# google/zopfli

Measured on AMD Instinct MI355X. Metric: input MB/s at numiterations=15 (gzip, bit-exact vs reference), higher is better.
Workload: dtype u8 (f32/f64 cost DP); 1 GPU; class-T synthetic (text-like, the enwik8 stand-in) 100000000 B per GPU, numiterations=15, blocksplitting=0, gzip, BASELINE configs[1]; total_bytes=100000000, master_blocks=100, gather=none (one rank)

## Files before the change

### zopfli_amd/csrc/device/drv_build.h

```cpp
#pragma once

constexpr u32 kMatchGrid = 1024;
constexpr u32 kMatchGrid5 = 1536;

extern "C" {
static unsigned SegL(u64 total_positions) {
  if (Knobs().seg_l_set) return Knobs().seg_l;
  total_positions = std::max<u64>(total_positions, zamd::CallPositions());
  return total_positions <= (128u << 10) ? 256u : total_positions <= (16u << 20) ? 512u : total_positions <= (48u << 20) ? 1024u : 2048u;
}
static unsigned SegHead(size_t nb) {
  const unsigned v = Knobs().seg_head;
  return v ? v : (nb >= 48 ? 8192u : 0u);
}


static int LayoutBlocks(zmx_ctx* c, const zmx_block* blocks, size_t nb, zmx_tables* t, u64* la_total, u64* max_window) {
  t->nb = nb;
  t->blocks.resize(nb);
  t->bsize.resize(nb);
  t->store_begin[0].assign(nb, 0);
  t->store_begin[1].assign(nb, 0);
  std::vector<u32> tile_off(nb + 1, 0);
  u64 pos_off = 0, reg_off = 0, la_off = 0, max_l = 0;
  for (size_t b = 0; b < nb; ++b) {
    if (blocks[b].inend < blocks[b].instart || blocks[b].inend > c->insize) {
      return FailMsg("zmx_tables_build: block outside the resident input");
    }
    BlockDesc& d = t->blocks[b];
    d.instart = blocks[b].instart;
    d.inend = blocks[b].inend;
    d.ws = d.instart > ZMX_WINDOW ? d.instart - ZMX_WINDOW : 0;
    if (!c->seg_starts.empty()) {
      const size_t k = static_cast<size_t>(std::upper_bound(c->seg_starts.begin(), c->seg_starts.end(), d.instart) -
                                           c->seg_starts.begin()) - 1;
      const u64 seg_end = k + 1 < c->seg_starts.size() ? c->seg_starts[k + 1] : c->insize;
      if (d.inend > seg_end) return FailMsg("zmx_tables_build: block spans two input segments (zmx_set_input_segments)");
      d.ws = std::max<u64>(d.ws, c->seg_starts[k]);
    }
    d.pos_off = pos_off;
    d.reg_off = reg_off;
    d.la_off = la_off;
    const u64 B = d.inend - d.instart, L = d.inend - d.ws;
    if (B > 0x7fff0000ull) return FailMsg("zmx_tables_build: block too large (positions are 32-bit)");
    t->bsize[b] = static_cast<u32>(B);
    pos_off += B;
    reg_off += (L + 7) & ~7ull;
    la_off += (B + 1 + 7) & ~7ull;
    max_l = std::max(max_l, L);
    tile_off[b + 1] = tile_off[b] + static_cast<u32>((B + MT - 1) / MT);
  }
  t->total_b = pos_off;
  t->total_l = reg_off;
  t->tile_off = tile_off;
  *la_total = la_off;
  *max_window = max_l;
  return 0;
}

struct ReusePlan {
  bool reuse = false;
  std::vector<u64> src_pos;
  std::vector<u64> link_lo;
  std::vector<u32> tile_list;
};
static ReusePlan PlanReuse(const zmx_ctx* c, const zmx_tables* t, const zmx_tables* parent, const std::vector<uint64_t>& tail_r) {
  const size_t nb = t->nb;
  const u64 pos_off = t->total_b;
  const std::vector<u32>& tile_off = t->tile_off;
  ReusePlan plan;
  bool reuse = parent != nullptr && parent->nb > 0 && (c->h_in != nullptr || tail_r.size() == nb) && parent->d_recs != nullptr &&
               parent->total_b + pos_off < (3ull << 30);
  if (reuse) {
    plan.src_pos.resize(nb);
    plan.link_lo.resize(nb);
    size_t pb = 0;
    for (size_t b = 0; b < nb && reuse; ++b) {
      const BlockDesc& d = t->blocks[b];
      while (pb < parent->nb && parent->blocks[pb].inend < d.inend) ++pb;
      if (pb == parent->nb || d.instart < parent->blocks[pb].instart || d.inend > parent->blocks[pb].inend) {
        reuse = false;
        break;
      }
      const BlockDesc& pd = parent->blocks[pb];
      plan.src_pos[b] = pd.pos_off + (d.instart - pd.instart);
      const u64 B = d.inend - d.instart;
      plan.link_lo[b] = d.inend - d.ws;
      if (B == 0 || d.inend == pd.inend) continue;
      u64 t0 = B > ZMX_MAX_MATCH ? d.inend - ZMX_MAX_MATCH : d.instart;
      const u64 r = c->h_in ? zamd::TailRunStart(c->h_in, d.instart, d.inend) : tail_r[b];
      if (r < t0) t0 = r;
      const u32 tile_first = static_cast<u32>((t0 - d.instart) / MT);
      for (u32 tile = tile_first; tile < tile_off[b + 1] - tile_off[b]; ++tile) {
        plan.tile_list.push_back(tile_off[b] + tile);
      }
      const u64 first_index = d.instart + static_cast<u64>(tile_first) * MT - d.ws;
      plan.link_lo[b] = first_index > ZMX_WINDOW ? first_index - ZMX_WINDOW : 0;
    }
  }
  plan.reuse = reuse;
  return plan;
}

static int TailRuns(zmx_ctx* c, const zmx_tables* t, std::vector<uint64_t>* r) {
  const size_t nb = t->nb;
  std::vector<uint64_t> blocks(2 * nb);
  for (size_t b = 0; b < nb; ++b) {
    blocks[2 * b] = t->blocks[b].instart;
    blocks[2 * b + 1] = t->blocks[b].inend;
  }
  PoolScope tmp(c);
  uint64_t* d_blocks = nullptr;
  uint64_t* d_r = nullptr;
  HIPCHK(tmp.Upload(&d_blocks, blocks.data(), 2 * nb, "d_blocks"));
  HIPCHK(tmp.AllocT(&d_r, nb, "d_r"));
  TailRunParams P;
  P.in = c->d_in;
  P.blocks = d_blocks;
  P.r = d_r;
  hipLaunchKernelGGL(k_tail_runs, dim3(static_cast<unsigned>(nb)), dim3(64), 0, c->stream, P);
  KCHK(c, "k_tail_runs");
  r->resize(nb);
  HIPCHK(hipMemcpyAsync(r->data(), d_r, nb * sizeof(uint64_t), hipMemcpyDeviceToHost, c->stream));
  HIPCHK(hipStreamSynchronize(c->stream));
  return 0;
}

static int AllocTableArrays(zmx_ctx* c, zmx_tables* t, u64 la_off) {
  const size_t nb = t->nb;
  const u64 pos_off = t->total_b;
  const u64 reg_off = t->total_l;
  const std::vector<u32>& tile_off = t->tile_off;
  HIPCHK(PoolAlloc(c, &t->d_blocks, nb));
  HIPCHK(PoolAlloc(c, &t->d_tile_off, nb + 1));
  HIPCHK(PoolAlloc(c, &t->d_same16, reg_off));
  HIPCHK(PoolAlloc(c, &t->d_links, reg_off));
  HIPCHK(PoolAlloc(c, &t->d_recs, pos_off * 8));
  HIPCHK(PoolAlloc(c, &t->d_la, la_off));
  HIPCHK(PoolAlloc(c, &t->d_store[0], pos_off));
  HIPCHK(PoolAlloc(c, &t->d_store[1], pos_off));
  t->run = RunLayout(nb);
  HIPCHK(PoolAlloc(c, &t->d_runin, t->run.in_bytes));
  HIPCHK(PoolAlloc(c, &t->d_runout, t->run.out_bytes));
  HIPCHK(c->pool.PinnedTake(&t->h_runin, t->run.in_bytes, &t->h_runin_cap));
  HIPCHK(c->pool.PinnedTake(&t->h_runout, t->run.out_bytes, &t->h_runout_cap));
  HIPCHK(hipMemsetAsync(t->run.stats(t->d_runout), 0, RunLayout::stats_and_flags_bytes(), c->stream));
  HIPCHK(PoolAlloc(c, &t->d_dph, pos_off));
  HIPCHK(PoolAlloc(c, &t->d_block_edges, nb));
  t->badpos_words = pos_off / 32 + 4;
  HIPCHK(PoolAlloc(c, &t->d_badpos, t->badpos_words));
  HIPCHK(PoolAlloc(c, &t->d_code_base, nb));
  HIPCHK(PoolAlloc(c, &t->d_wtab, nb * ZMX_WTAB));
  HIPCHK(PoolAlloc(c, &t->d_badcodes, nb * 40));
  HIPCHK(PoolAlloc(c, &t->d_counters, 48));
  HIPCHK(hipMemcpyAsync(t->d_blocks, t->blocks.data(), nb * sizeof(BlockDesc), hipMemcpyHostToDevice, c->stream));
  HIPCHK(hipMemcpyAsync(t->d_tile_off, tile_off.data(), (nb + 1) * sizeof(u32), hipMemcpyHostToDevice, c->stream));
  HIPCHK(hipMemsetAsync(t->run.flags(t->d_runout), 0, RunLayout::kFlags * sizeof(u32), c->stream));
  return 0;
}

struct MatchBuild {
  PoolScope hash_tmp;
  u16* d_lev = nullptr;
  u16* d_tot2 = nullptr;
  u16* d_rank2 = nullptr;
  uint4* d_xrec = nullptr;
  u32* d_tot12 = nullptr;
  unsigned long long* d_energy = nullptr;
  u32* d_cmax = nullptr;
  u8* d_est = nullptr;
  bool skip_any = false, skip_all = false;
  double skip_positions = 0;
  unsigned long long* d_m5stats = nullptr;
  bool join_stream2 = false;
  explicit MatchBuild(zmx_ctx* c) : hash_tmp(c) {}
};

static int LaunchHash(zmx_ctx* c, zmx_tables* t, int mk, u64 max_l, const u64* d_link_lo, MatchBuild& m) {
  const size_t nb = t->nb;
  const u64 reg_off = t->total_l;
  if (max_l == 0) return 0;
  const dim3 g1(static_cast<unsigned>((max_l + 256 * SAME_CH - 1) / (256 * SAME_CH)), static_cast<unsigned>(nb));
  hipLaunchKernelGGL(k_same, g1, dim3(256), 0, c->stream, c->d_in, t->d_blocks, t->d_same16, d_link_lo);
  KCHK(c, "k_same");
  const dim3 g2(static_cast<unsigned>((max_l + CH_EMIT - 1) / CH_EMIT), static_cast<unsigned>(nb), 2);
  hipLaunchKernelGGL(k_chain, g2, dim3(64), CH_LDS_BYTES, c->stream, c->d_in, t->d_blocks, t->d_same16, t->d_links, d_link_lo);
  KCHK(c, "k_chain");
  const bool walks = mk == 5 || mk == 0;
  const bool order = mk != 5 && MatchOrder();
  if ((walks || order) && d_link_lo == nullptr) {
    m.skip_any = mk == 5;
    if (mk == 5) for (size_t b = 0; b < nb; ++b) m.skip_positions += static_cast<double>(t->blocks[b].inend - t->blocks[b].instart);
    const unsigned hits_chunks = static_cast<unsigned>((max_l + RK_CH - 1) / RK_CH);
    {
      if (!m.d_energy) HIPCHK(m.hash_tmp.AllocT(&m.d_energy, nb, "d_energy"));
      if (walks && !m.d_cmax) HIPCHK(m.hash_tmp.AllocT(&m.d_cmax, nb * static_cast<size_t>(hits_chunks) + 1, "d_cmax"));
      if (order && !m.d_est) HIPCHK(m.hash_tmp.AllocT(&m.d_est, reg_off, "d_est"));
      HIPCHK(hipMemsetAsync(m.d_energy, 0, nb * sizeof(unsigned long long), c->stream));
      if (m.d_cmax) HIPCHK(hipMemsetAsync(m.d_cmax, 0, (nb * static_cast<size_t>(hits_chunks) + 1) * sizeof(u32), c->stream));
      HitsParams hp;
      hp.in = c->d_in;
      hp.blocks = t->d_blocks;
      hp.same16 = t->d_same16;
      hp.energy = m.d_energy;
      hp.cmax = m.d_cmax;
      hp.est = m.d_est;
      const dim3 g5(hits_chunks, static_cast<unsigned>(nb));
      hipLaunchKernelGGL(k_hits, g5, dim3(RK_THREADS), 0, c->stream, hp);
      KCHK(c, "k_hits");
    }
    if (!walks) return 0;
    if (mk == 0) {
      std::vector<unsigned long long> energy(nb);
      HIPCHK(hipMemcpyAsync(energy.data(), m.d_energy, nb * sizeof(unsigned long long), hipMemcpyDeviceToHost, c->stream));
      HIPCHK(hipStreamSynchronize(c->stream));
      size_t on = 0;
      for (size_t b = 0; b < nb; ++b) {
        if (energy[b] > Knobs().match_hits * (t->blocks[b].inend - t->blocks[b].ws)) {
          ++on;
          m.skip_positions += static_cast<double>(t->blocks[b].inend - t->blocks[b].instart);
        }
      }
      m.skip_any = on != 0;
      m.skip_all = on == nb;
    }
    if (m.skip_any) {
      if (!m.d_lev) HIPCHK(m.hash_tmp.AllocT(&m.d_lev, static_cast<size_t>(LV_N) * reg_off, "d_lev"));
      if (!m.d_tot2) HIPCHK(m.hash_tmp.AllocT(&m.d_tot2, 2 * reg_off, "d_tot"));
      if (!m.d_rank2) HIPCHK(m.hash_tmp.AllocT(&m.d_rank2, 2 * reg_off, "d_rank"));
      if (!m.d_tot12) HIPCHK(m.hash_tmp.AllocT(&m.d_tot12, reg_off, "d_tot12"));
      if (!m.d_xrec) HIPCHK(m.hash_tmp.AllocT(&m.d_xrec, 2 * reg_off, "d_xrec"));
      LevelParams lp;
      lp.in = c->d_in;
      lp.blocks = t->d_blocks;
      lp.lev = m.d_lev;
      lp.total_l = reg_off;
      lp.energy = mk == 0 ? m.d_energy : nullptr;
      lp.thr = Knobs().match_hits;
      const dim3 g4(static_cast<unsigned>((max_l + LV_CH - 1) / LV_CH), static_cast<unsigned>(nb), LV_N);
      hipLaunchKernelGGL(k_levels, g4, dim3(64), 0, c->stream, lp);
      KCHK(c, "k_levels");
      RankParams rp;
      rp.in = c->d_in;
      rp.blocks = t->d_blocks;
      rp.links = t->d_links;
      rp.same16 = t->d_same16;
      rp.lev = m.d_lev;
      rp.total_l = reg_off;
      rp.tot = m.d_tot2;
      rp.rank = m.d_rank2;
      rp.xrec = m.d_xrec;
      rp.tot12 = m.d_tot12;
      rp.energy = lp.energy;
      rp.thr = lp.thr;
      rp.cmax = m.d_cmax;
      rp.cmax_stride = hits_chunks;
      const dim3 g3(static_cast<unsigned>((max_l + RK_CH - 1) / RK_CH), static_cast<unsigned>(nb));
      hipLaunchKernelGGL(k_rank2, g3, dim3(RK_THREADS), 0, c->stream, rp);
      KCHK(c, "k_rank2");
    }
  }
  return 0;
}
static int BuildHashLinks(zmx_ctx* c, zmx_tables* t, int mk, u64 max_l, const ReusePlan& plan, MatchBuild& m) {
  const size_t nb = t->nb;
  HIPCHK(hipEventRecord(c->ev[0], c->stream));
  u64* d_link_lo = nullptr;
  if (plan.reuse) HIPCHK(m.hash_tmp.Upload(&d_link_lo, plan.link_lo.data(), nb, "d_link_lo"));
  if (LaunchHash(c, t, mk, max_l, d_link_lo, m) != 0) return -1;
  t->links_partial = plan.reuse;
  return 0;
}

static int LaunchMatch(zmx_ctx* c, zmx_tables* t, int mk, MatchBuild& m, u32* pool, u32 pool_cap, u32 total_tiles, const u32* d_tiles, bool prof) {
  const size_t nb = t->nb;
  if (total_tiles == 0) return 0;
  MatchParams mp;
  mp.in = c->d_in;
  mp.blocks = t->d_blocks;
  mp.tile_off = t->d_tile_off;
  mp.nb = static_cast<u32>(nb);
  mp.total_tiles = total_tiles;
  mp.links = t->d_links;
  mp.recs = t->d_recs;
  mp.pool = pool;
  mp.pool_cap = pool_cap;
  mp.counters = t->d_counters;
  mp.scratch = c->d_scratch;
  mp.tile_list = d_tiles;
  mp.skip_energy = nullptr;
  mp.skip_thr = 0;
  mp.est = d_tiles == nullptr ? m.d_est : nullptr;
  if ((mk == 5 || mk == 0) && d_tiles == nullptr && m.skip_any) {
    if (!c->d_scratch5) HIPCHK(PoolAllocT(c, &c->d_scratch5, static_cast<size_t>(kMatchGrid5) * M5_THREADS * SCRATCH_CPS, "d_scratch5"));
    Match5Params q;
    q.m = mp;
    q.m.scratch = c->d_scratch5;
    q.xrec = m.d_xrec;
    q.tot12 = m.d_tot12;
    q.energy = mk == 0 ? m.d_energy : nullptr;
    q.thr = Knobs().match_hits;
    const size_t m5_waves = static_cast<size_t>(kMatchGrid5) * (M5_THREADS / 64);
    if (!m.d_m5stats) HIPCHK(m.hash_tmp.AllocT(&m.d_m5stats, 2 * m5_waves, "d_m5stats"));
    HIPCHK(hipMemsetAsync(m.d_m5stats, 0, 2 * m5_waves * sizeof(unsigned long long), c->stream));
    q.wave_stats = m.d_m5stats;
    {
      const u64 waves = static_cast<u64>(kMatchGrid5) * (M5_THREADS / 64);
      q.sub_shift = mp.total_tiles >= 4 * waves ? 1u : 2u;
    }
    if (mk == 5 || m.skip_all) {
      hipLaunchKernelGGL(k_match5, dim3(kMatchGrid5), dim3(M5_THREADS), 0, c->stream, q);
      KCHK(c, "k_match5");
      return 0;
    }
    HIPCHK(hipEventRecord(c->ev2[0], c->stream));
    HIPCHK(hipStreamWaitEvent(c->stream2, c->ev2[0], 0));
    hipLaunchKernelGGL(k_match5, dim3(kMatchGrid5), dim3(M5_THREADS), 0, c->stream2, q);
    HIPCHK(hipGetLastError());
    c->stream2_outstanding = true;
    HIPCHK(hipEventRecord(c->ev2[1], c->stream2));
    m.join_stream2 = true;
    mp.skip_energy = m.d_energy;
    mp.skip_thr = Knobs().match_hits;
  }
  const bool filt = Knobs().match_filter;
  if (prof && filt) hipLaunchKernelGGL((k_match2<true, true>), dim3(kMatchGrid), dim3(M2_THREADS), 0, c->stream, mp);
  else if (prof) hipLaunchKernelGGL((k_match2<true, false>), dim3(kMatchGrid), dim3(M2_THREADS), 0, c->stream, mp);
  else if (filt) hipLaunchKernelGGL((k_match2<false, true>), dim3(kMatchGrid), dim3(M2_THREADS), 0, c->stream, mp);
  else hipLaunchKernelGGL((k_match2<false, false>), dim3(kMatchGrid), dim3(M2_THREADS), 0, c->stream, mp);
  if (m.join_stream2) {
    m.join_stream2 = false;
    HIPCHK(hipStreamWaitEvent(c->stream, c->ev2[1], 0));
    c->stream2_outstanding = false;
  }
  KCHK(c, "k_match2");
  return 0;
}

static int BuildMatchRecords(zmx_ctx* c, zmx_tables* t, zmx_tables* parent, int mk, u64 max_l, const ReusePlan& plan, MatchBuild& m) {
  const size_t nb = t->nb;
  const u64 pos_off = t->total_b;
  const std::vector<u32>& tile_off = t->tile_off;
  bool reuse = plan.reuse;
  if (!c->d_scratch) HIPCHK(PoolAllocT(c, &c->d_scratch, static_cast<size_t>(kMatchGrid) * M2_THREADS * SCRATCH_CPS, "d_scratch"));
  HIPCHK(hipEventRecord(c->ev[1], c->stream));
  double match_positions = 0;
  double m5_lane_iters = 0, m5_iters = 0;
  if (reuse) {
    u64* d_src_pos = nullptr;
    u32* d_tile_list = nullptr;
    PoolScope tmp(c);
    HIPCHK(tmp.Upload(&d_src_pos, plan.src_pos.data(), nb, "d_src_pos"));
    HIPCHK(tmp.Upload(&d_tile_list, plan.tile_list.data(), plan.tile_list.size(), "d_tile_list"));
    CopyRecsParams cp;
    cp.blocks = t->d_blocks;
    cp.src_pos = d_src_pos;
    cp.src = reinterpret_cast<const uint4*>(parent->d_recs);
    cp.dst = reinterpret_cast<uint4*>(t->d_recs);
    u64 max_b = 0;
    for (size_t b = 0; b < nb; ++b) max_b = std::max<u64>(max_b, t->bsize[b]);
    const unsigned gx = static_cast<unsigned>(std::min<u64>(std::max<u64>((max_b * 2 + 256 * 16 - 1) / (256 * 16), 1), 4096));
    hipLaunchKernelGGL(k_copy_recs, dim3(gx, static_cast<unsigned>(nb)), dim3(256), 0, c->stream, cp);
    KCHK(c, "k_copy_recs");
    HIPCHK(hipMemsetAsync(t->d_counters, 0, 48 * sizeof(u32), c->stream));
    HIPCHK(hipMemcpyAsync(t->d_counters, parent->d_counters, sizeof(u32), hipMemcpyDeviceToDevice, c->stream));
    if (LaunchMatch(c, t, mk, m, parent->d_pool, parent->pool_cap, static_cast<u32>(plan.tile_list.size()), d_tile_list, false) != 0) return -1;
    u32 counters[2] = {0, 0};
    HIPCHK(hipMemcpyAsync(counters, t->d_counters, sizeof(counters), hipMemcpyDeviceToHost, c->stream));
    HIPCHK(hipStreamSynchronize(c->stream));
    if ((counters[1] & 1u) == 0) {
      t->d_pool = parent->d_pool;
      t->pool_cap = parent->pool_cap;
      parent->d_pool = nullptr;
      parent->pool_cap = 0;
      parent->params.trace.pool = nullptr;
    } else {
      reuse = false;
      if (LaunchHash(c, t, mk, max_l, nullptr, m) != 0) return -1;
      t->links_partial = false;
    }
  }

  const u64 pool_entries = Knobs().pool_entries;
  u64 per_pos = 4;
  for (bool first_try = true; !reuse; first_try = false) {
    u64 cap = std::max<u64>(pos_off * per_pos, 1u << 16);
    if (first_try && pool_entries) cap = pool_entries;
    if (cap > 0xfffffff0ull) cap = 0xfffffff0ull;
    PoolFree(c, t->d_pool);
    t->d_pool = nullptr;
    HIPCHK(PoolAlloc(c, &t->d_pool, cap));
    t->pool_cap = static_cast<u32>(cap);
    HIPCHK(hipMemsetAsync(t->d_counters, 0, 48 * sizeof(u32), c->stream));
    if (LaunchMatch(c, t, mk, m, t->d_pool, t->pool_cap, tile_off[nb], nullptr, Knobs().prof) != 0) return -1;
    u32 counters[2] = {0, 0};
    HIPCHK(hipMemcpyAsync(counters, t->d_counters, sizeof(counters), hipMemcpyDeviceToHost, c->stream));
    HIPCHK(hipStreamSynchronize(c->stream));
    match_positions += static_cast<double>(pos_off);
    if (m.d_m5stats) {
      const size_t m5_waves = static_cast<size_t>(kMatchGrid5) * (M5_THREADS / 64);
      std::vector<unsigned long long> ws(2 * m5_waves);
      HIPCHK(hipMemcpy(ws.data(), m.d_m5stats, ws.size() * sizeof(unsigned long long), hipMemcpyDeviceToHost));
      m5_lane_iters = m5_iters = 0;
      for (size_t w = 0; w < m5_waves; ++w) { m5_lane_iters += static_cast<double>(ws[2 * w]); m5_iters += static_cast<double>(ws[2 * w + 1]); }
    }
    if (counters[1] & 2u) {
      u32 dbg[8] = {0};
      HIPCHK(hipMemcpy(dbg, t->d_counters + 32, sizeof(dbg), hipMemcpyDeviceToHost));
      char buf[320];
      std::snprintf(buf, sizeof(buf), "zmx_tables_build: k_match5's wave loop did not end (state %08x xd %u curd %u bestlen %u limit %u nlink %u eqd %u "
                    "li %u idx %u same %u cur %u bestdist %u)", dbg[0], dbg[1], dbg[2], dbg[3] & 0xffffu, dbg[3] >> 16, dbg[4] & 0xffffu, dbg[4] >> 16,
                    dbg[5], dbg[6] & 0xffffu, dbg[6] >> 16, dbg[7] & 0xffffu, dbg[7] >> 16);
      return FailFault(buf);
    }
    if ((counters[1] & 1u) == 0) break;
    if (per_pos >= 256) return FailMsg("zmx_tables_build: change-point pool overflow");
    per_pos *= 8;
  }
  {
    HIPCHK(hipEventRecord(c->ev[2], c->stream));
    HIPCHK(hipEventSynchronize(c->ev[2]));
    float ms_hash = 0, ms_match = 0;
    HIPCHK(hipEventElapsedTime(&ms_hash, c->ev[0], c->ev[1]));
    HIPCHK(hipEventElapsedTime(&ms_match, c->ev[1], c->ev[2]));
    zmx_stats& ts = zamd::ThreadStats();
    ts.match[0] += ms_match * 1e-3;
    ts.match[1] += ms_hash * 1e-3;
    ts.match[2] += 1;
    ts.match[3] += reuse ? static_cast<double>(plan.tile_list.size()) * MT : match_positions;
    if (m.skip_any && !reuse) {
      ts.match5[0] += m5_lane_iters;
      ts.match5[1] += m5_iters;
      ts.match5[2] += m.skip_positions;
    }
    if (Knobs().prof && !reuse) {
      unsigned long long hc[2] = {0, 0};
      HIPCHK(hipMemcpy(hc, t->d_counters + 4, sizeof(hc), hipMemcpyDeviceToHost));
      const double pos = static_cast<double>(pos_off);
      std::fprintf(stderr, "%s: %.2f ms for %.0f positions: %.1f chain hits per "
                   "position, %.1f of 64 lanes with a hit per wave-loop iteration; %.1f SIMD cycles per hit (2.4 GHz, 1024 SIMDs)\n", mk == 5 || mk == 0 ? "k_match5 / k_match2 (hits = entries touched)" : "k_match2", ms_match, pos,
                   static_cast<double>(hc[0]) / pos, static_cast<double>(hc[0]) / static_cast<double>(hc[1] ? hc[1] : 1),
                   ms_match * 1e-3 * 2.4e9 * 1024 / static_cast<double>(hc[0] ? hc[0] : 1));
      if (mk != 5) {
        int wgs = 0;
        if (Knobs().match_filter) HIPCHK(hipOccupancyMaxActiveBlocksPerMultiprocessor(&wgs, k_match2<false, true>, M2_THREADS, 0));
        else HIPCHK(hipOccupancyMaxActiveBlocksPerMultiprocessor(&wgs, k_match2<false, false>, M2_THREADS, 0));
        std::fprintf(stderr, "k_match2: %d workgroups of %u threads resident per CU; positions handed out %s\n", wgs, M2_THREADS,
                     m.d_est ? "by k_hits' estimate, longest first" : "in ascending order");
      }
    }
  }
  return 0;
}

static int BuildDpRows(zmx_ctx* c, zmx_tables* t) {
  const size_t nb = t->nb;
  const std::vector<u32>& tile_off = t->tile_off;
  RowScanParams rp;
  rp.blocks = t->d_blocks;
  rp.recs = t->d_recs;
  rp.dph = t->d_dph;
  rp.block_edges = t->d_block_edges;
  rp.codeless = !Knobs().run_codes && SegL(t->total_b) != 0 ? 1u : 0u;
  hipLaunchKernelGGL(k_rowscan, dim3(static_cast<unsigned>(nb)), dim3(1024), 0, c->stream, rp);
  KCHK(c, "k_rowscan");
  t->block_edges.resize(nb);
  HIPCHK(hipMemcpyAsync(t->block_edges.data(), t->d_block_edges, nb * sizeof(u64), hipMemcpyDeviceToHost, c->stream));
  HIPCHK(hipStreamSynchronize(c->stream));
  {
    const u64 env_mb = Knobs().code_budget_mb;
    const u64 budget = (env_mb ? env_mb * (1ull << 20) : static_cast<u64>(c->code_budget)) / sizeof(u16);
    std::vector<u64> code_base(nb, 0);
    u64 cur = 0;
    for (size_t b = 0; b < nb; ++b) {
      if (t->block_edges[b] > 0xffff0000ull) return FailMsg("zmx_tables_build: block too large (DP row offsets are 32-bit)");
      code_base[b] = cur;
      cur += ((t->block_edges[b] + DP_PIECE - 1) & ~static_cast<u64>(DP_PIECE - 1)) + DP_PIECE;
    }
    if (cur > budget && nb > 1) {
      return FailTooLarge("zmx_tables_build: the batch needs more room for its DP edges than ZOPFLI_AMD_CODE_BUDGET_MB allows");
    }
    HIPCHK(PoolAlloc(c, &t->d_codes, cur + 2048));
    HIPCHK(hipMemcpyAsync(t->d_code_base, code_base.data(), nb * sizeof(u64), hipMemcpyHostToDevice, c->stream));
    CodeParams kp;
    kp.blocks = t->d_blocks;
    kp.tile_off = t->d_tile_off;
    kp.nb_total = static_cast<u32>(nb);
    kp.recs = t->d_recs;
    kp.pool = t->d_pool;
// ... 312 lines not shown
```

### zopfli_amd/csrc/device/zmx_kernels.h

```cpp
#pragma once
#include <hip/hip_runtime.h>
#include <stdint.h>

#include "zmx_record.h"

typedef unsigned char u8;
typedef unsigned short u16;
typedef unsigned int u32;
typedef unsigned long long u64;

struct BlockDesc {
  u64 instart, inend, ws;
  u64 pos_off;
  u64 reg_off;
  u64 la_off;
};

#define ZMX_WINDOW 32768u
#define ZMX_MAX_MATCH 258u
#define ZMX_MAX_CHAIN_HITS 8192
#define ZMX_NONE16 0xffffu

__device__ __forceinline__ int dev_dist_symbol(u32 d) {
  if (d < 5) return (int)d - 1;
  const int l = 31 - __clz((int)(d - 1));
  return 2 * l + (int)(((d - 1) >> (l - 1)) & 1);
}
__device__ __forceinline__ int dev_dist_extra_bits(u32 d) {
  return d < 5 ? 0 : (31 - __clz((int)(d - 1))) - 1;
}
__device__ __forceinline__ int dev_length_symbol(u32 l) {
  if (l < 11) return 254 + (int)l;
  if (l == 258) return 285;
  const int e = 31 - __clz((int)(l - 3)) - 2;
  return 261 + 4 * e + (int)(((l - 3) >> e) & 3);
}
__device__ __forceinline__ int dev_length_extra_bits(u32 l) {
  if (l < 11 || l == 258) return 0;
  return 31 - __clz((int)(l - 3)) - 2;
}

__device__ __forceinline__ u32 find_block(const u32* off, u32 n, u32 x) {
  u32 lo = 0, hi = n;
  while (hi - lo > 1) {
    const u32 mid = (lo + hi) >> 1;
    if (off[mid] <= x) lo = mid; else hi = mid;
  }
  return lo;
}

#define ZMX_WAVE_SCAN(NAME, OP, IDENT)                                                   \
  __device__ __forceinline__ u32 NAME(u32 v) {                                           \
    u32 t;                                                                               \
    t = (u32)__builtin_amdgcn_update_dpp((int)(IDENT), (int)v, 0x111, 0xf, 0xf, false); v = OP(v, t); \
    t = (u32)__builtin_amdgcn_update_dpp((int)(IDENT), (int)v, 0x112, 0xf, 0xf, false); v = OP(v, t); \
    t = (u32)__builtin_amdgcn_update_dpp((int)(IDENT), (int)v, 0x114, 0xf, 0xf, false); v = OP(v, t); \
    t = (u32)__builtin_amdgcn_update_dpp((int)(IDENT), (int)v, 0x118, 0xf, 0xf, false); v = OP(v, t); \
    t = (u32)__builtin_amdgcn_update_dpp((int)(IDENT), (int)v, 0x142, 0xa, 0xf, false); v = OP(v, t); \
    t = (u32)__builtin_amdgcn_update_dpp((int)(IDENT), (int)v, 0x143, 0xc, 0xf, false); v = OP(v, t); \
    return v;                                                                            \
  }
__device__ __forceinline__ u32 zmx_addu(u32 a, u32 b) { return a + b; }
__device__ __forceinline__ u32 zmx_maxu(u32 a, u32 b) { return a > b ? a : b; }
ZMX_WAVE_SCAN(wave_scan_add, zmx_addu, 0u)
ZMX_WAVE_SCAN(wave_scan_max, zmx_maxu, 0u)

__device__ __forceinline__ u32 rdlane_u32(u32 v, u32 l) { return (u32)__builtin_amdgcn_readlane((int)v, (int)l); }
__device__ __forceinline__ float rdlane_f32(float v, u32 l) {
  return __int_as_float(__builtin_amdgcn_readlane(__float_as_int(v), (int)l));
}
__device__ __forceinline__ void wave_lds_sync() {
  __builtin_amdgcn_fence(__ATOMIC_ACQ_REL, "wavefront");
  __builtin_amdgcn_wave_barrier();
}

#define SAME_CH 64

__global__ __launch_bounds__(256) void k_same(const u8* __restrict__ in, const BlockDesc* __restrict__ blocks,
                                              u16* __restrict__ same16, const u64* __restrict__ link_lo) {
  const BlockDesc bd = blocks[blockIdx.y];
  const u64 L = bd.inend - bd.ws;
  const u64 c0 = ((u64)blockIdx.x * blockDim.x + threadIdx.x) * SAME_CH;
  if (c0 >= L) return;
  const u64 c1 = (c0 + SAME_CH < L) ? c0 + SAME_CH : L;
  if (link_lo) {
    const u64 lo = link_lo[blockIdx.y];
    if (lo >= L) return;
    const u64 chunk0 = lo / 32768u * 32768u;
    if (c1 + 32768u <= chunk0) return;
  }
  const u8* base = in + bd.ws;
  u32 next = 0;
  if (c1 < L) {
    const u8 c = base[c1];
    u64 q = c1 + 1;
    u32 r = 0;
    bool stop = false;
    while (q < L && r < 65535u && (((u64)(base + q)) & 7)) {
      if (base[q] != c) { stop = true; break; }
      ++q; ++r;
    }
    if (!stop) {
      const u64 pat = 0x0101010101010101ull * c;
      while (q + 8 <= L && r < 65535u) {
        const u64 x = *reinterpret_cast<const u64*>(base + q) ^ pat;
        if (x) { r += (u32)(__ffsll((long long)x) - 1) >> 3; stop = true; break; }
        q += 8; r += 8;
      }
      if (!stop) {
        while (q < L && r < 65535u && base[q] == c) { ++q; ++r; }
      }
    }
    next = r < 65535u ? r : 65535u;
  }
  u16* out = same16 + bd.reg_off;
  for (u64 k = c1; k-- > c0;) {
    u32 s = 0;
    if (k + 1 < L && base[k + 1] == base[k]) s = next < 65535u ? next + 1 : 65535u;
    out[k] = (u16)s;
    next = s;
  }
}

#define CH_EMIT 32768u
#define CH_TILE 1024u
#define CH_LDS_BYTES (65536 + CH_TILE * 4)

__global__ __launch_bounds__(64) void k_chain(const u8* __restrict__ in, const BlockDesc* __restrict__ blocks,
                                              const u16* __restrict__ same16, ushort4* __restrict__ links,
                                              const u64* __restrict__ link_lo) {
  extern __shared__ __align__(16) u8 dyn_lds[];
  u16* head = reinterpret_cast<u16*>(dyn_lds);
  u16* keys = head + 32768;
  u16* sames = keys + CH_TILE;

  const BlockDesc bd = blocks[blockIdx.y];
  const u32 chain = blockIdx.z;
  const u64 L = bd.inend - bd.ws;
  const u64 e0 = (u64)blockIdx.x * CH_EMIT;
  if (e0 >= L) return;
  const u64 e1 = (e0 + CH_EMIT < L) ? e0 + CH_EMIT : L;
  if (link_lo && e1 <= link_lo[blockIdx.y]) return;
  const u64 w0 = e0 >= ZMX_WINDOW ? e0 - ZMX_WINDOW : 0;
  const u32 lane = threadIdx.x;
  const u64 lt_mask = (1ull << lane) - 1;
  const u64 gt_mask = ~((2ull << lane) - 1);

  for (u32 i = lane; i < 16384; i += 64) reinterpret_cast<u32*>(head)[i] = 0xffffffffu;
  __syncthreads();

  const u8* base = in + bd.ws;
  const u16* same = same16 + bd.reg_off;
  ushort4* lk = links + bd.reg_off;

  for (u64 t0 = w0; t0 < e1; t0 += CH_TILE) {
    const u32 tn = (u32)((e1 - t0 < CH_TILE) ? e1 - t0 : CH_TILE);
    {
      const u32 i0 = 16u * lane;
      u32 by[18];
      u32 sm[16];
#pragma unroll
      for (u32 q = 0; q < 18; ++q) {
        const u64 k = t0 + i0 + q;
        by[q] = (i0 < tn && k < L) ? (u32)base[k] : 0u;
      }
#pragma unroll
      for (u32 q = 0; q < 16; ++q) sm[q] = (i0 + q < tn) ? (u32)same[t0 + i0 + q] : 0u;
#pragma unroll
      for (u32 q = 0; q < 16; ++q) {
        if (i0 + q < tn) {
          u32 v = ((by[q] << 10) ^ (by[q + 1] << 5) ^ by[q + 2]) & 32767u;
          if (chain) v ^= (sm[q] - 3u) & 255u;
          keys[i0 + q] = (u16)v;
          sames[i0 + q] = (u16)sm[q];
        }
      }
    }
    __syncthreads();
    const u32 cur0 = (u32)(t0 - w0);
    for (u32 i0 = 0; i0 < tn; i0 += 64) {
      const u32 i = i0 + lane;
      const bool act = i < tn;
      const u32 key = act ? (u32)keys[i] : 0u;
      if (t0 + i0 + 64 <= e0) {
        const u32 r = cur0 + i;
        bool todo = act;
        while (__any(todo)) {
          if (todo) head[key] = (u16)r;
          wave_lds_sync();
          const u32 w = act ? (u32)head[key] : 0xffffu;
          wave_lds_sync();
          todo = act && w < r;
        }
        continue;
      }
      const u32 old = act ? (u32)head[key] : (u32)ZMX_NONE16;
      u64 grp = __ballot(act);
#pragma unroll
      for (int bit = 0; bit < 15; ++bit) {
        const bool mine = (key >> bit) & 1;
        const u64 bm = __ballot(mine);
        grp &= mine ? bm : ~bm;
      }
      const u64 lower = grp & lt_mask;
      const u32 r = cur0 + i;
      u32 d;
      if (lower) d = lane - (63u - (u32)__clzll((long long)lower));
      else d = old == ZMX_NONE16 ? 0u : r - old;
      if (d > 32767u) d = 0;
      wave_lds_sync();
      if (act && (grp & gt_mask) == 0) head[key] = (u16)r;
      wave_lds_sync();
      const u64 k = t0 + i;
      if (act && k >= e0) {
        if (chain == 0) {
          lk[k].x = (u16)d;
          lk[k].z = sames[i];
        } else {
          lk[k].y = (u16)d;
        }
      }
    }
    __syncthreads();
  }
}

#ifndef MT
#define MT 2048u
#endif
#define MWIN_BYTES (32768u + MT + 288u)
#define SCRATCH_CPS 256u
#ifndef M_XCD_GROUP
#define M_XCD_GROUP 16u
#endif
#ifndef MATCH_BATCH
#define MATCH_BATCH 8u
#endif

struct MatchParams {
  const u8* in;
  const BlockDesc* blocks;
  const u32* tile_off;
  u32 nb;
  u32 total_tiles;
  const ushort4* links;
  u32* recs;
  u32* pool;
  u32 pool_cap;
  u32* counters;
  u32* scratch;
  const u32* tile_list;
  const unsigned long long* skip_energy;
  u64 skip_thr;
  const u8* est = nullptr;
};

__device__ __forceinline__ u32 lds_byte(const u32* w, u32 a) { return reinterpret_cast<const u8*>(w)[a]; }
__device__ __forceinline__ u32 lds_u32_unaligned(const u32* w, u32 a) {
  const u32 lo = w[a >> 2], hi = w[(a >> 2) + 1];
  return __builtin_amdgcn_alignbyte(hi, lo, a & 3);
}

template <class First8>
__device__ __forceinline__ bool rec_pool_claim(const MatchParams& P, u32 ncp, const u32* scratch, First8 first8, u32& off) {
  off = atomicAdd(&P.counters[0], ncp);
  if (off + ncp <= P.pool_cap) {
#pragma unroll
    for (u32 e = 0; e < zamd::kRecInlineCps; ++e) P.pool[off + e] = first8(e);
    for (u32 e = zamd::kRecInlineCps; e < ncp; ++e) P.pool[off + e] = scratch[e];
    return true;
  }
  atomicOr(&P.counters[1], 1u);
  return false;
}

struct CopyRecsParams {
  const BlockDesc* blocks;
  const u64* src_pos;
  const uint4* src;
  uint4* dst;
};

__global__ __launch_bounds__(256) void k_copy_recs(CopyRecsParams P) {
  const BlockDesc bd = P.blocks[blockIdx.y];
  const u64 n = (u64)(bd.inend - bd.instart) * 2;
  const uint4* src = P.src + P.src_pos[blockIdx.y] * 2;
  uint4* dst = P.dst + bd.pos_off * 2;
  for (u64 i = (u64)blockIdx.x * 256 + threadIdx.x; i < n; i += (u64)gridDim.x * 256) dst[i] = src[i];
}

__device__ __forceinline__ void hist_add_symbol(u32* hist, u32 litlen, u32 dist) {
  if (dist == 0) {
    atomicAdd(&hist[litlen], 1u);
  } else {
    atomicAdd(&hist[dev_length_symbol(litlen)], 1u);
    atomicAdd(&hist[288 + dev_dist_symbol(dist)], 1u);
  }
}

__device__ __forceinline__ uint2 greedy_window(const u32* rbase, u32 wb, u32 lane, u32 B) {
  const u32 q = wb + lane < B ? wb + lane : (B ? B - 1 : 0);
  return *reinterpret_cast<const uint2*>(rbase + (u64)q * 8);
}

#define TR_CHUNK 2048u

struct RowScanParams {
  const BlockDesc* blocks;
  const u32* recs;
  uint2* dph;
  u64* block_edges;
  u32 codeless;
};
#define DPH_CODELESS (1u << 26)
__device__ __forceinline__ u32 dph_layout_len(u32 y) { return (y & DPH_CODELESS) ? 0u : (y & 0xffffu); }

__global__ __launch_bounds__(1024) void k_rowscan(RowScanParams P) {
  __shared__ u32 s_wsum[16];
  const BlockDesc bd = P.blocks[blockIdx.x];
  const u32 B = (u32)(bd.inend - bd.instart);
  const u32 tid = threadIdx.x, lane = tid & 63, wid = tid >> 6;
  const u32* rbase = P.recs + bd.pos_off * 8;
  uint2* out = P.dph + bd.pos_off;
  u64 carry = 0;
  for (u32 t0 = 0; t0 < B; t0 += 1024) {
    const u32 jj = t0 + tid;
    const bool act = jj < B;
    u32 kend = 0, sflag = 0;
    if (act) {
      const uint2 h = *reinterpret_cast<const uint2*>(rbase + (u64)jj * 8);
      const u32 leng = zamd::RecLength(h.x), dist = zamd::RecDist(h.x), same_i = zamd::RecSame(h.y), ncp = zamd::RecCount(h.y);
      if (leng >= 3 && dist == 1u && ncp == 1u) sflag |= 2u;
      sflag |= zamd::RecLiteral(h.y) << 2;
      kend = leng < B - jj ? leng : B - jj;
      if (kend < 3) kend = 1;
      if (same_i > 2 * ZMX_MAX_MATCH && jj > ZMX_MAX_MATCH + 1 && jj + 2 * ZMX_MAX_MATCH + 1 < B) {
        const u32 same_back = zamd::RecSame(rbase[(u64)(jj - ZMX_MAX_MATCH) * 8 + 1]);
        sflag |= same_back > ZMX_MAX_MATCH ? 1u : 0u;
      }
    }
    const bool nocodes = P.codeless != 0 && (sflag & 2u) != 0 && kend >= 64u;
    const u32 klay = nocodes ? 0u : kend;
    const u32 incl = wave_scan_add(klay);
    if (lane == 63) s_wsum[wid] = incl;
    __syncthreads();
    u32 woff = 0, tot = 0;
#pragma unroll
    for (u32 w = 0; w < 16; ++w) {
      const u32 v = s_wsum[w];
      if (w < wid) woff += v;
      tot += v;
    }
    if (act) out[jj] = make_uint2((u32)carry + woff + incl - klay, kend | (sflag << 16) | (nocodes ? DPH_CODELESS : 0u));
    carry += tot;
    __syncthreads();
  }
  if (tid == 0) P.block_edges[blockIdx.x] = carry;
}

#define EG_CAP 2048u
#define ZMX_NUM_W 1127u
#define ZMX_WTAB 1152u

__device__ __forceinline__ u32 weight_code(u32 k, u32 dist) {
  return (257u + 30u * (u32)(dev_length_symbol(k) - 257) + (u32)dev_dist_symbol(dist)) * 8u;
}

struct CodeParams {
  const BlockDesc* blocks;
  const u32* tile_off;
  u32 nb_total;
  const u32* recs;
  const u32* pool;
  const uint2* dph;
  u16* codes;
  const u64* code_base;
};

__global__ __launch_bounds__(256) void k_codes(CodeParams P) {
  __shared__ u8 s_mark[4][EG_CAP];
  __shared__ u32 s_hoff[4][64];
  __shared__ u32 s_hthr[4][64][2];
  __shared__ u16 s_hdist[4][64][8];
  __shared__ u32 s_hpool[4][64][2];

  const u32 tid = threadIdx.x, lane = tid & 63, wid = tid >> 6;
  const u32 tile = blockIdx.x;
  const u32 b = find_block(P.tile_off, P.nb_total, tile);
  const BlockDesc bd = P.blocks[b];
  const u32 B = (u32)(bd.inend - bd.instart);
  const u32 tp0 = (tile - P.tile_off[b]) * MT;
  const u32* rbase = P.recs + bd.pos_off * 8;
  const uint2* dbase = P.dph + bd.pos_off;
  u16* codes = P.codes + P.code_base[b];
  u8* mark = s_mark[wid];

  for (u32 g = wid; g < MT / 64; g += 4) {
    const u32 base = tp0 + g * 64;
    if (base >= B) break;
    const u32 navail = (B - base < 64u) ? B - base : 64u;
    const u32 jj = base + lane;
    const bool act = lane < navail;
    uint4 ra = make_uint4(0, 0, 0, 0), rb = make_uint4(0, 0, 0, 0);
    uint2 dh = make_uint2(0, 0);
    if (act) {
      ra = *reinterpret_cast<const uint4*>(rbase + (u64)jj * 8);
      rb = *reinterpret_cast<const uint4*>(rbase + (u64)jj * 8 + 4);
      dh = dbase[jj];
    }
    const u32 lit = zamd::RecLiteral(ra.y);
    const u32 ncpf = zamd::RecCount(ra.y);
    const u32 kend = dh.y & 0xffffu;
    const u32 klay = dph_layout_len(dh.y);
    const u32 off = dh.x;
    const u32 offend = off + (act ? klay : 0u);
    const u32 off0 = rdlane_u32(off, 0);

    wave_lds_sync();
    {
      const bool ovf = ncpf == zamd::kRecOverflow;
      s_hoff[wid][lane] = (off - off0) | (lit << 16) | ((ovf ? 1u : 0u) << 24);
      if (ovf) {
        s_hpool[wid][lane][0] = zamd::RecPoolOffset(ra.z);
        s_hpool[wid][lane][1] = zamd::RecPoolCount(ra.w);
        s_hthr[wid][lane][0] = 0xffffffffu;
        s_hthr[wid][lane][1] = 0xffffffffu;
      } else {
        const u32 w[6] = {ra.z, ra.w, rb.x, rb.y, rb.z, rb.w};
        u32 t0 = 0, t1 = 0;
#pragma unroll
        for (int e = 0; e < 8; ++e) {
          const u32 v = zamd::RecCpFieldOfWords(w, (u32)e);
          zamd::RecCpThresholdPut(t0, t1, (u32)e, ncpf, v);
          s_hdist[wid][lane][e] = (u16)zamd::RecCpDist(v);
        }
        s_hthr[wid][lane][0] = t0;
        s_hthr[wid][lane][1] = t1;
      }
    }

    u32 q = 0;
    while (q < navail) {
      const u32 off_q = rdlane_u32(off, q);
      const u64 fit = __ballot(act && lane >= q && offend - off_q <= EG_CAP);
      const u32 n = (u32)__popcll(fit);
      const u32 E = rdlane_u32(offend, q + n - 1) - off_q;
      wave_lds_sync();
      for (u32 e = lane; e < (E + 3) / 4; e += 64) reinterpret_cast<u32*>(mark)[e] = 0;
      wave_lds_sync();
      if (lane >= q && lane < q + n && klay != 0) mark[off - off_q] = (u8)(lane + 1);
      wave_lds_sync();
      const u32 rel_q = off_q - off0;
      u32 carry = q + 1;
      u64 ovf_mask = __ballot(lane >= q && lane < q + n && ncpf == zamd::kRecOverflow);
      for (u32 t0 = 0; t0 < E; t0 += 64) {
        const u32 e = t0 + lane;
        const u32 mk = e < E ? (u32)mark[e] : 0u;
        u32 own = wave_scan_max(mk);
        own = own > carry ? own : carry;
        carry = rdlane_u32(own, 63);
        if (e < E) {
          const u32 p = own - 1;
          const u32 h = s_hoff[wid][p];
          const u32 k = e - ((h & 0xffffu) - rel_q) + 1;
          u32 code;
          if (k == 1) {
            code = (1u + ((h >> 16) & 255u)) * 8u;
          } else if (k == 2 || (h >> 24)) {
            code = 0;
          } else {
            const u32 idx = zamd::RecCpThresholdIndex(s_hthr[wid][p][0], s_hthr[wid][p][1], k - 3);
            code = weight_code(k, s_hdist[wid][p][idx]);
          }
          codes[(u64)off_q + e] = (u16)code;
        }
      }
      while (ovf_mask) {
        const u32 p = (u32)__ffsll((long long)ovf_mask) - 1;
        ovf_mask &= ovf_mask - 1;
        const u32 roff_p = rdlane_u32(off, p);
        const u32 ke = rdlane_u32(kend, p);
        const u32 poff = s_hpool[wid][p][0], pn = s_hpool[wid][p][1];
        for (u32 k = 3 + lane; k <= ke; k += 64) {
          const u32 plo = zamd::RecPoolFind(P.pool, poff, pn, k);
          const u32 dist = plo < pn ? zamd::RecPoolDist(P.pool[poff + plo]) : 1u;
          codes[(u64)roff_p + k - 1] = (u16)weight_code(k, dist);
        }
      }
      q += n;
    }
  }
}

struct WtabParams {
  const double* cost;
  const double* mincost;
  double* wtab;
  u32* badcodes;
  u32* stats;
};

__global__ __launch_bounds__(256) void k_wtab(WtabParams P) {
  __shared__ u32 s_bad[40];
  const u32 b = blockIdx.x, tid = threadIdx.x;
  if (tid < 40) s_bad[tid] = 0;
  if (b == 0 && tid < ZMX_SEG_N && P.stats) P.stats[tid] = 0;
  __syncthreads();
  const double* ll = P.cost + (u64)b * 320;
  const double* d = ll + 288;
  const double mincost = P.mincost[b];
  for (u32 c = tid; c < ZMX_WTAB; c += 256) {
    double w = __longlong_as_double(0x7ff0000000000000ll);
    if (c >= 1 && c <= 256) {
      w = ll[c - 1];
    } else if (c >= 257 && c < ZMX_NUM_W) {
      const u32 ls = 257u + (c - 257u) / 30u, ds = (c - 257u) % 30u;
      const int lb = ls < 265 || ls == 285 ? 0 : (int)(ls - 261) / 4;
      const int db = ds < 4 ? 0 : (int)ds / 2 - 1;
      w = ((double)(lb + db) + ll[ls]) + d[ds];
      if (w < mincost) {
        atomicAdd(&s_bad[0], 1u);
        atomicOr(&s_bad[4 + (c >> 5)], 1u << (c & 31));
      }
    }
    P.wtab[(u64)b * ZMX_WTAB + c] = w;
  }
  __syncthreads();
// ... 98 lines not shown
```

Before: 930.7 MB/s.

## Rebuild hash-chain kernel with multi-wave key partitioning and atomicMax head updates

k_chain moves from a single 64-thread wave to 8 waves. Each wave owns a partition of hash keys and queues its positions in a per-wave LDS ring, then processes rounds of 256 entries. It uses atomicMax on 32-bit heads with ballot-based group detection, replacing the 15-ballot key compare and the retry loop. It also prefetches the next tile's input into registers while the current tile is processed. The aim is to spread the serial chain-link construction across more waves per workgroup. In exchange the kernel is more complex, needs more LDS per block, and still has to produce exactly the same links for bit-exact output.

```diff
diff --git a/zopfli_amd/csrc/device/drv_build.h b/zopfli_amd/csrc/device/drv_build.h
--- a/zopfli_amd/csrc/device/drv_build.h
+++ b/zopfli_amd/csrc/device/drv_build.h
@@ -184,7 +184,7 @@
   hipLaunchKernelGGL(k_same, g1, dim3(256), 0, c->stream, c->d_in, t->d_blocks, t->d_same16, d_link_lo);
   KCHK(c, "k_same");
   const dim3 g2(static_cast<unsigned>((max_l + CH_EMIT - 1) / CH_EMIT), static_cast<unsigned>(nb), 2);
-  hipLaunchKernelGGL(k_chain, g2, dim3(64), CH_LDS_BYTES, c->stream, c->d_in, t->d_blocks, t->d_same16, t->d_links, d_link_lo);
+  hipLaunchKernelGGL(k_chain, g2, dim3(zamd::kHlThreads), CH_LDS_BYTES, c->stream, c->d_in, t->d_blocks, t->d_same16, t->d_links, d_link_lo);
   KCHK(c, "k_chain");
   const bool walks = mk == 5 || mk == 0;
   const bool order = mk != 5 && MatchOrder();
diff --git a/zopfli_amd/csrc/device/zmx_hashlink_rules.h b/zopfli_amd/csrc/device/zmx_hashlink_rules.h
--- /dev/null
+++ b/zopfli_amd/csrc/device/zmx_hashlink_rules.h
@@ -0,0 +1,76 @@
+#ifndef ZMX_HASHLINK_RULES_H_
+#define ZMX_HASHLINK_RULES_H_
+
+#include <stdint.h>
+
+#if defined(__HIPCC__)
+#define ZMX_HL_HD __host__ __device__
+#else
+#define ZMX_HL_HD
+#endif
+
+#ifndef CH_EMIT
+#define CH_EMIT 32768u
+#endif
+#ifndef HL_WAVES
+#define HL_WAVES 8u
+#endif
+
+namespace zamd {
+
+constexpr uint32_t kHlWindow = 32768;
+constexpr uint32_t kHlEmit = CH_EMIT;
+constexpr uint32_t kHlKeys = 32768;
+constexpr uint32_t kHlKeyBits = 15, kHlPosBits = 17;
+constexpr uint32_t kHlWaves = HL_WAVES;
+constexpr uint32_t kHlThreads = 64 * kHlWaves;
+constexpr uint32_t kHlLoad = kHlWaves <= 4 ? 16 : 8;
+constexpr uint32_t kHlTile = kHlThreads * kHlLoad;
+constexpr uint32_t kHlSteps = 4;
+constexpr uint32_t kHlRound = 64 * kHlSteps;
+constexpr uint32_t kHlBatch = 256;
+constexpr uint32_t kHlQueue = 512;
+
+static_assert(kHlEmit % kHlWindow == 0 && kHlEmit >= kHlWindow, "the emitted chunk is a multiple of 32768");
+static_assert(kHlWindow + kHlEmit <= (1u << kHlPosBits), "a job position has 17 bits");
+static_assert((kHlWaves & (kHlWaves - 1)) == 0 && kHlWaves >= 1 && kHlWaves <= 16, "the partition is a mask of key bits");
+static_assert(kHlTile % kHlBatch == 0 && kHlWindow % kHlTile == 0, "tiles start at multiples of the batch; a chunk at a tile");
+static_assert((kHlQueue & (kHlQueue - 1)) == 0 && kHlRound - 1 + kHlBatch <= kHlQueue, "the ring never wraps onto itself");
+
+constexpr uint32_t kHlLdsBytes = kHlKeys * 4 + kHlTile * 2 * 2 + kHlWaves * kHlQueue * 4;
+static_assert(kHlLdsBytes <= 160 * 1024, "one workgroup on a CU's 160 KiB");
+
+ZMX_HL_HD inline uint32_t HlKey(uint32_t b0, uint32_t b1, uint32_t b2) { return ((b0 << 10) ^ (b1 << 5) ^ b2) & 32767u; }
+ZMX_HL_HD inline uint32_t HlKey2(uint32_t key, uint32_t same) { return key ^ ((same - 3u) & 255u); }
+
+ZMX_HL_HD inline uint32_t HlPartition(uint32_t key) { return (key ^ (key >> 5) ^ (key >> 10)) & (kHlWaves - 1u); }
+
+ZMX_HL_HD inline uint32_t HlEntry(uint32_t key, uint32_t jobpos) { return key << kHlPosBits | jobpos; }
+ZMX_HL_HD inline uint32_t HlEntryKey(uint32_t e) { return e >> kHlPosBits; }
+ZMX_HL_HD inline uint32_t HlEntryPos(uint32_t e) { return e & ((1u << kHlPosBits) - 1u); }
+
+ZMX_HL_HD inline uint32_t HlQueueSlot(uint32_t head, uint32_t i) { return (head + i) & (kHlQueue - 1u); }
+
+struct HlJob {
+  uint64_t w0;
+  uint32_t nw;
+  uint32_t n;
+};
+ZMX_HL_HD inline HlJob HlJobOf(uint64_t chunk, uint64_t L) {
+  const uint64_t e0 = chunk * kHlEmit;
+  const uint64_t e1 = e0 + kHlEmit < L ? e0 + kHlEmit : L;
+  HlJob j;
+  j.nw = e0 >= kHlWindow ? kHlWindow : 0u;
+  j.w0 = e0 - j.nw;
+  j.n = static_cast<uint32_t>(e1 - j.w0);
+  return j;
+}
+
+ZMX_HL_HD inline bool HlRoundReady(uint32_t count) { return count >= kHlRound; }
+ZMX_HL_HD inline bool HlRoundWarmOnly(uint32_t last_jobpos, uint32_t nw) { return last_jobpos < nw; }
+
+ZMX_HL_HD inline uint64_t HlFirstChunkStart(uint64_t link_lo) { return link_lo / kHlEmit * kHlEmit; }
+
+}
+
+#endif
diff --git a/zopfli_amd/csrc/device/zmx_kernels.h b/zopfli_amd/csrc/device/zmx_kernels.h
--- a/zopfli_amd/csrc/device/zmx_kernels.h
+++ b/zopfli_amd/csrc/device/zmx_kernels.h
@@ -2,6 +2,7 @@
 #include <hip/hip_runtime.h>
 #include <stdint.h>
 
+#include "zmx_hashlink_rules.h"
 #include "zmx_record.h"
 
 typedef unsigned char u8;
@@ -86,8 +87,8 @@
   if (link_lo) {
     const u64 lo = link_lo[blockIdx.y];
     if (lo >= L) return;
-    const u64 chunk0 = lo / 32768u * 32768u;
-    if (c1 + 32768u <= chunk0) return;
+    const u64 chunk0 = zamd::HlFirstChunkStart(lo);
+    if (c1 + zamd::kHlWindow <= chunk0) return;
   }
   const u8* base = in + bd.ws;
   u32 next = 0;
@@ -122,107 +123,177 @@
   }
 }
 
-#define CH_EMIT 32768u
-#define CH_TILE 1024u
-#define CH_LDS_BYTES (65536 + CH_TILE * 4)
-
-__global__ __launch_bounds__(64) void k_chain(const u8* __restrict__ in, const BlockDesc* __restrict__ blocks,
-                                              const u16* __restrict__ same16, ushort4* __restrict__ links,
-                                              const u64* __restrict__ link_lo) {
+#define CH_LDS_BYTES zamd::kHlLdsBytes
+
+struct ChStage {
+  u32 by[zamd::kHlLoad + 2];
+  u32 sm[zamd::kHlLoad];
+};
+__device__ __forceinline__ void ch_load(ChStage& st, const u8* base, const u16* same, u64 t0, u32 tn, u64 L, u32 i0) {
+#pragma unroll
+  for (u32 q = 0; q < zamd::kHlLoad + 2; ++q) {
+    const u64 k = t0 + i0 + q;
+    st.by[q] = (i0 < tn && k < L) ? (u32)base[k] : 0u;
+  }
+#pragma unroll
+  for (u32 q = 0; q < zamd::kHlLoad; ++q) st.sm[q] = (i0 + q < tn) ? (u32)same[t0 + i0 + q] : 0u;
+}
+
+template <bool GUARD>
+__device__ __forceinline__ void ch_round(const u32* ring, u32* head, u32 qhead, u32 cnt, u32 nw, u32 chain, ushort4* lkw,
+                                         u32 lane, u64 lt_mask) {
+  u32 key[zamd::kHlSteps], q[zamd::kHlSteps];
+#pragma unroll
+  for (u32 u = 0; u < zamd::kHlSteps; ++u) {
+    const u32 e = ring[zamd::HlQueueSlot(qhead, 64u * u + lane)];
+    key[u] = zamd::HlEntryKey(e);
+    q[u] = zamd::HlEntryPos(e);
+  }
+  if (!GUARD && zamd::HlRoundWarmOnly(rdlane_u32(q[zamd::kHlSteps - 1], 63), nw)) {
+#pragma unroll
+    for (u32 u = 0; u < zamd::kHlSteps; ++u) atomicMax(&head[key[u]], q[u] + 1u);
+    return;
+  }
+  u32 old[zamd::kHlSteps], ret[zamd::kHlSteps];
+#pragma unroll
+  for (u32 u = 0; u < zamd::kHlSteps; ++u) {
+    old[u] = 0;
+    ret[u] = 0;
+    if (!GUARD || 64u * u + lane < cnt) {
+      old[u] = head[key[u]];
+      ret[u] = atomicMax(&head[key[u]], q[u] + 1u);
+    }
+  }
+  u64 grp[zamd::kHlSteps];
+#pragma unroll
+  for (u32 u = 0; u < zamd::kHlSteps; ++u) {
+    const bool act = !GUARD || 64u * u + lane < cnt;
+    const u32 step0 = rdlane_u32(q[u], 0) + 1u;
+    u64 F = __ballot(act && ret[u] >= step0);
+    grp[u] = 0;
+    while (F) {
+      const u32 l0 = (u32)__ffsll((unsigned long long)F) - 1u;
+      const u32 k0 = rdlane_u32(key[u], l0);
+      const bool mine = act && key[u] == k0;
+      const u64 G = __ballot(mine);
+      if (mine) grp[u] = G;
+      F &= ~G;
+    }
+  }
+  u32 qs[zamd::kHlSteps];
+#pragma unroll
+  for (u32 u = 0; u < zamd::kHlSteps; ++u) {
+    const u64 lower = grp[u] & lt_mask;
+    const u32 src = lower ? 63u - (u32)__clzll((long long)lower) : lane;
+    qs[u] = (u32)__shfl((int)q[u], (int)src);
+  }
+#pragma unroll
+  for (u32 u = 0; u < zamd::kHlSteps; ++u) {
+    const bool act = !GUARD || 64u * u + lane < cnt;
+    u32 d = old[u] ? q[u] + 1u - old[u] : 0u;
+    if (grp[u] & lt_mask) d = q[u] - qs[u];
+    if (d > 32767u) d = 0;
+    if (act && q[u] >= nw) {
+      if (chain == 0) lkw[q[u]].x = (u16)d; else lkw[q[u]].y = (u16)d;
+    }
+  }
+}
+
+__global__ __launch_bounds__(zamd::kHlThreads) void k_chain(const u8* __restrict__ in, const BlockDesc* __restrict__ blocks,
+                                                            const u16* __restrict__ same16, ushort4* __restrict__ links,
+                                                            const u64* __restrict__ link_lo) {
   extern __shared__ __align__(16) u8 dyn_lds[];
-  u16* head = reinterpret_cast<u16*>(dyn_lds);
-  u16* keys = head + 32768;
-  u16* sames = keys + CH_TILE;
+  u32* head = reinterpret_cast<u32*>(dyn_lds);
+  u16* keys = reinterpret_cast<u16*>(head + zamd::kHlKeys);
+  u16* sames = keys + zamd::kHlTile;
+  u32* rings = reinterpret_cast<u32*>(sames + zamd::kHlTile);
 
   const BlockDesc bd = blocks[blockIdx.y];
   const u32 chain = blockIdx.z;
   const u64 L = bd.inend - bd.ws;
   const u64 e0 = (u64)blockIdx.x * CH_EMIT;
   if (e0 >= L) return;
-  const u64 e1 = (e0 + CH_EMIT < L) ? e0 + CH_EMIT : L;
+  const zamd::HlJob job = zamd::HlJobOf(blockIdx.x, L);
+  const u64 w0 = job.w0, e1 = job.w0 + job.n;
   if (link_lo && e1 <= link_lo[blockIdx.y]) return;
-  const u64 w0 = e0 >= ZMX_WINDOW ? e0 - ZMX_WINDOW : 0;
-  const u32 lane = threadIdx.x;
+  const u32 tid = threadIdx.x;
+  const u32 lane = tid & 63u;
+  const u32 wave = (u32)__builtin_amdgcn_readfirstlane((int)(tid >> 6));
   const u64 lt_mask = (1ull << lane) - 1;
-  const u64 gt_mask = ~((2ull << lane) - 1);
-
-  for (u32 i = lane; i < 16384; i += 64) reinterpret_cast<u32*>(head)[i] = 0xffffffffu;
-  __syncthreads();
+  u32* ring = rings + wave * zamd::kHlQueue;
 
   const u8* base = in + bd.ws;
   const u16* same = same16 + bd.reg_off;
   ushort4* lk = links + bd.reg_off;
-
-  for (u64 t0 = w0; t0 < e1; t0 += CH_TILE) {
-    const u32 tn = (u32)((e1 - t0 < CH_TILE) ? e1 - t0 : CH_TILE);
-    {
-      const u32 i0 = 16u * lane;
-      u32 by[18];
-      u32 sm[16];
-#pragma unroll
-      for (u32 q = 0; q < 18; ++q) {
-        const u64 k = t0 + i0 + q;
-        by[q] = (i0 < tn && k < L) ? (u32)base[k] : 0u;
-      }
-#pragma unroll
-      for (u32 q = 0; q < 16; ++q) sm[q] = (i0 + q < tn) ? (u32)same[t0 + i0 + q] : 0u;
-#pragma unroll
-      for (u32 q = 0; q < 16; ++q) {
-        if (i0 + q < tn) {
-          u32 v = ((by[q] << 10) ^ (by[q + 1] << 5) ^ by[q + 2]) & 32767u;
-          if (chain) v ^= (sm[q] - 3u) & 255u;
-          keys[i0 + q] = (u16)v;
-          sames[i0 + q] = (u16)sm[q];
+  ushort4* lkw = lk + w0;
+  const u32 i0 = zamd::kHlLoad * tid;
+
+  ChStage st;
+  u64 t0 = w0;
+  u32 tn = (u32)((e1 - t0 < zamd::kHlTile) ? e1 - t0 : zamd::kHlTile);
+  ch_load(st, base, same, t0, tn, L, i0);
+  for (u32 i = tid; i < zamd::kHlKeys / 4; i += zamd::kHlThreads) reinterpret_cast<uint4*>(head)[i] = make_uint4(0, 0, 0, 0);
+
+  u32 qhead = 0, qcount = 0;
+  for (;;) {
+#pragma unroll
+    for (u32 q = 0; q < zamd::kHlLoad; ++q) {
+      if (i0 + q < tn) {
+        u32 v = zamd::HlKey(st.by[q], st.by[q + 1], st.by[q + 2]);
+        if (chain) v = zamd::HlKey2(v, st.sm[q]);
+        keys[i0 + q] = (u16)v;
+        sames[i0 + q] = (u16)st.sm[q];
+      }
+    }
+    __syncthreads();
+    const u64 t1 = t0 + zamd::kHlTile;
+    const bool more = t1 < e1;
+    u32 tn1 = 0;
+    if (more) {
+      tn1 = (u32)((e1 - t1 < zamd::kHlTile) ? e1 - t1 : zamd::kHlTile);
+      ch_load(st, base, same, t1, tn1, L, i0);
+    }
+    if (chain == 0) {
+      for (u32 i = tid; i < tn; i += zamd::kHlThreads) {
+        if (t0 + i >= e0) lk[t0 + i].z = sames[i];
+      }
+    }
+    const u32 cur0 = (u32)(t0 - w0);
+    for (u32 g = 0; g < tn; g += zamd::kHlBatch) {
+      u32 kk[zamd::kHlBatch / 64];
+      u64 m[zamd::kHlBatch / 64];
+#pragma unroll
+      for (u32 u = 0; u < zamd::kHlBatch / 64; ++u) {
+        const u32 i = g + 64u * u + lane;
+        kk[u] = i < tn ? (u32)keys[i] : 0xffffffffu;
+      }
+#pragma unroll
+      for (u32 u = 0; u < zamd::kHlBatch / 64; ++u) m[u] = __ballot(kk[u] != 0xffffffffu && zamd::HlPartition(kk[u]) == wave);
+      u64 any = 0;
+#pragma unroll
+      for (u32 u = 0; u < zamd::kHlBatch / 64; ++u) any |= m[u];
+      if (any == 0) continue;
+#pragma unroll
+      for (u32 u = 0; u < zamd::kHlBatch / 64; ++u) {
+        if ((m[u] >> lane) & 1) {
+          ring[zamd::HlQueueSlot(qhead, qcount + (u32)__popcll(m[u] & lt_mask))] = zamd::HlEntry(kk[u], cur0 + g + 64u * u + lane);
         }
-      }
-    }
+        qcount += (u32)__popcll(m[u]);
+      }
+      wave_lds_sync();
+      while (zamd::HlRoundReady(qcount)) {
+        ch_round<false>(ring, head, qhead, qcount, job.nw, chain, lkw, lane, lt_mask);
+        qhead = zamd::HlQueueSlot(qhead, zamd::kHlRound);
+        qcount -= zamd::kHlRound;
+      }
+      wave_lds_sync();
+    }
+    if (!more) break;
     __syncthreads();
-    const u32 cur0 = (u32)(t0 - w0);
-    for (u32 i0 = 0; i0 < tn; i0 += 64) {
-      const u32 i = i0 + lane;
-      const bool act = i < tn;
-      const u32 key = act ? (u32)keys[i] : 0u;
-      if (t0 + i0 + 64 <= e0) {
-        const u32 r = cur0 + i;
-        bool todo = act;
-        while (__any(todo)) {
-          if (todo) head[key] = (u16)r;
-          wave_lds_sync();
-          const u32 w = act ? (u32)head[key] : 0xffffu;
-          wave_lds_sync();
-          todo = act && w < r;
-        }
-        continue;
-      }
-      const u32 old = act ? (u32)head[key] : (u32)ZMX_NONE16;
-      u64 grp = __ballot(act);
-#pragma unroll
-      for (int bit = 0; bit < 15; ++bit) {
-        const bool mine = (key >> bit) & 1;
-        const u64 bm = __ballot(mine);
-        grp &= mine ? bm : ~bm;
-      }
-      const u64 lower = grp & lt_mask;
-      const u32 r = cur0 + i;
-      u32 d;
-      if (lower) d = lane - (63u - (u32)__clzll((long long)lower));
-      else d = old == ZMX_NONE16 ? 0u : r - old;
-      if (d > 32767u) d = 0;
-      wave_lds_sync();
-      if (act && (grp & gt_mask) == 0) head[key] = (u16)r;
-      wave_lds_sync();
-      const u64 k = t0 + i;
-      if (act && k >= e0) {
-        if (chain == 0) {
-          lk[k].x = (u16)d;
-          lk[k].z = sames[i];
-        } else {
-          lk[k].y = (u16)d;
-        }
-      }
-    }
-    __syncthreads();
-  }
+    t0 = t1;
+    tn = tn1;
+  }
+  if (qcount) ch_round<true>(ring, head, qhead, qcount, job.nw, chain, lkw, lane, lt_mask);
 }
 
 #ifndef MT
```

Result: no change. 933.5 MB/s (median of 2 runs) (+0.3%).
